# simplify23/TPS_PP

Hardware: AMD Instinct MI355X
Metric: rectified images/sec (3x32x100) (higher is better)
Workload: dtype f32; 1 GPU; BASELINE.json configs[1]: fused TPS grid-gen + bilinear grid_sample HIP kernel, batch 512 per GPU, 3x32x100 fp32, 20 fiducials, inputs resident in HBM; batch_per_gpu=512, rotating_buffer_sets=14, streams=3, repeats=1

## Files before the change

tps_pp_amd/csrc/tpspp_warp_pair.h:

```cpp
#pragma once
#include "tpspp_warp_dev.h"

namespace tpspp_pair {

using namespace tpspp_dev;

typedef float v4f __attribute__((ext_vector_type(4)));
typedef float v4f_a4 __attribute__((ext_vector_type(4), aligned(4)));
typedef __attribute__((address_space(1))) char gchar;

struct PairParams {
    const float* in; const float* ctrl; const float* inv_delta_c;
    const float* packed;
    const float* p_hat;
    int p_hat_ld;
    int N;
    float* out; float* grid; int32_t* idx;
    int zero_off;
    int out_off;
    long long* trace;
};

template <int F>
__device__ __forceinline__ constexpr int perm_y(int k) { return (k + F / 2) % F; }
template <int F>
__device__ __forceinline__ constexpr int perm_x(int k) { return k < F / 2 ? F / 2 - 1 - k : F + F / 2 - 1 - k; }

__device__ __forceinline__ void store16_nt(gchar* p, v4f v)
{
    asm volatile("global_store_dwordx4 %0, %1, off nt\n\ts_nop 1" ::"v"(p), "v"(v) : "memory");
}

__device__ __forceinline__ void wait_flag(const float* flag_word, int want)
{
    const volatile int* f = reinterpret_cast<const volatile int*>(flag_word);
    while (*f < want) __builtin_amdgcn_s_sleep(1);
}
__device__ __forceinline__ void wait_flag_lds(const float* flag_word, int want)
{
    typedef __attribute__((address_space(3))) const volatile int lds_cvint;
    lds_cvint* f = (lds_cvint*)(size_t)(unsigned)(size_t)flag_word;
    while (__builtin_amdgcn_readfirstlane(*f) < want) __builtin_amdgcn_s_sleep(1);
}

template <int OFF>
__device__ __forceinline__ void flag_add(unsigned addr, int one)
{
    asm volatile("ds_add_u32 %0, %1 offset:%2" ::"v"(addr), "v"(one), "n"(OFF) : "memory");
}

struct TapsLite {
    int o00;
    float nw, ne, sw, se;
    float wx, wy;
    bool inx, iny;
    int x0, y0;
};
__device__ __forceinline__ TapsLite make_taps_lite(float gx, float gy, int H, int W)
{
    TapsLite t;
    const float limx = (float)(W - 1), limy = (float)(H - 1);
    float ix = (gx + 1.0f) * (0.5f * limx);
    float iy = (gy + 1.0f) * (0.5f * limy);
    ix = (ix > 0.0f) ? ix : 0.0f;
    iy = (iy > 0.0f) ? iy : 0.0f;
    ix = __builtin_fminf(ix, limx);
    iy = __builtin_fminf(iy, limy);
    const float w = __builtin_amdgcn_fractf(ix), nn = __builtin_amdgcn_fractf(iy);
    int x0, y0;
    asm("v_cvt_flr_i32_f32 %0, %1" : "=v"(x0) : "v"(ix));
    asm("v_cvt_flr_i32_f32 %0, %1" : "=v"(y0) : "v"(iy));
    const float e = 1.0f - w, s = 1.0f - nn;
    t.nw = s * e; t.ne = s * w; t.sw = nn * e; t.se = nn * w;
    t.wx = w; t.wy = nn;
    t.inx = ix < limx;
    t.iny = iy < limy;
    t.o00 = __mul24(y0, W) + x0;
    t.x0 = x0; t.y0 = y0;
    return t;
}

template <int F, int q>
__device__ __forceinline__ void mirror_vals(const float* v_row, float (&val)[4])
{
    if constexpr (q == 0) {
        val[0] = val[1] = val[2] = val[3] = v_row[0];
    } else if constexpr (q == 1) {
        val[0] = v_row[1]; val[1] = -v_row[1]; val[2] = v_row[1]; val[3] = -v_row[1];
    } else if constexpr (q == 2) {
        val[0] = v_row[2]; val[1] = v_row[2]; val[2] = -v_row[2]; val[3] = -v_row[2];
    } else {
        constexpr int k = q - 3;
        val[0] = v_row[3 + k];
        val[1] = v_row[3 + perm_x<F>(k)];
        val[2] = v_row[3 + perm_y<F>(k)];
        val[3] = v_row[3 + perm_x<F>(perm_y<F>(k))];
    }
}

constexpr int kPairFlags = 4;
constexpr int kPairLoaders = 3;
constexpr int kPairAwait = 6;
constexpr int kPairKB = 4;

constexpr int kPairVarPacked = 1;
constexpr int kPairVarMfma = 2;
typedef float v2f __attribute__((ext_vector_type(2)));

template <int OH, int OW>
struct PairGeo {
    static constexpr int halfW = OW / 2;
    static constexpr int PW = (halfW + 3) & ~3;
    static constexpr int CGP = PW / 4;
    static constexpr int CG = (halfW - 2) / 4;
    static constexpr int SC0 = CG * 4;
    static constexpr int SW = OW - 2 * SC0;
    static constexpr int nthr = (OH / 2) * CG * 4;
    static constexpr int NW = nthr / kWave;
    static_assert(OW % 4 == 0 && (OH / 2) % 8 == 0 && nthr % kWave == 0, "needs whole 4 x 8 pixel blocks, whole wavefronts");
    static_assert(SW == 4 && OH * SW == 2 * kWave, "the centre strip is 4 columns, two wavefronts per image");
    static_assert(NW % 4 == 0 && NW >= 4, "the compute wavefronts spread evenly over the four SIMDs");
};
__host__ __device__ inline void pair_thread_pixel(int t, int CG, int* r, int* c)
{
    const int hw = t >> 5, l5 = t & 31, rg = hw / CG, cg = hw - rg * CG;
    *r = rg * 8 + (l5 >> 2);
    *c = cg * 4 + (l5 & 3);
}

template <int F, int C, int HC, int WC, int OH, int OW, bool AUX, bool TRACE, int VAR = 0>
__global__ void __launch_bounds__(1024)
tps_warp_pair_kernel(const PairParams P)
{
    using Geo = PairGeo<OH, OW>;
    constexpr int K = F + 3;
    constexpr int H = HC, W = WC;
    constexpr int NW = Geo::NW, NLOAD = kPairLoaders;
    constexpr int n = OH * OW;
    static_assert(NW + NLOAD <= 16, "too many wavefronts");
    extern __shared__ __attribute__((aligned(16))) float smem[];
    float4* sT = reinterpret_cast<float4*>(smem);
    float* sFlag = smem + 4 * K + 2 * ((K * K + 3) & ~3);
    float* sImg = sFlag + kPairFlags;
    float* sZero = sImg + P.zero_off;
    float* sOut = sImg + P.out_off;

    const int tid = threadIdx.x;
    const int lane = tid & (kWave - 1);
    const int wv = __builtin_amdgcn_readfirstlane(tid / kWave);
    const int b0 = blockIdx.x * 2;
    const bool hasB = (b0 + 1) < P.N;
    constexpr int HW = H * W;
    constexpr int img_elems = C * HW;

    unsigned ts[8];
#define PAIR_STAMP(i) do { if (TRACE) ts[i] = (unsigned)__builtin_amdgcn_s_memtime(); } while (0)
    long long wall0 = 0;
    if (TRACE) wall0 = (long long)wall_clock64();
    PAIR_STAMP(7);

    constexpr int KGI = (K + 3) / 4;
    float hrowv[KGI * 4];
    float cx = 0.0f, cy = 0.0f;
    if (wv < 2) {
        if (lane < F) {
            const int b = (wv == 1 && hasB) ? b0 + 1 : b0;
            const float2 cc = reinterpret_cast<const float2*>(P.ctrl + (size_t)b * F * 2)[lane];
            cx = cc.x; cy = cc.y;
        }
        const float* row = P.inv_delta_c + (lane < K ? lane : K - 1) * K;
#pragma unroll
        for (int j = 0; j < KGI; ++j) {
            const int c0 = (j == KGI - 1) ? K - 4 : 4 * j;
            const v4f_a4 x = *reinterpret_cast<const v4f_a4*>(row + c0);
            hrowv[4 * j] = x[0]; hrowv[4 * j + 1] = x[1]; hrowv[4 * j + 2] = x[2]; hrowv[4 * j + 3] = x[3];
        }
    }
    if (tid < kPairFlags) reinterpret_cast<int*>(sFlag)[tid] = 0;
    lds_only_barrier();

    if (wv >= NW) {
        const int lw = wv - NW;
        const int total_bytes = (hasB ? 2 : 1) * img_elems * 4;
        const int pieces = (total_bytes + 1023) >> 10;
        const int piecesA = (img_elems * 4 + 1023) >> 10;
        const char* src = reinterpret_cast<const char*>(P.in + (size_t)b0 * img_elems);
        auto dma = [&](int piece) {
            int off = piece * 1024 + lane * 16;
            if (off >= total_bytes) off = 0;
            __builtin_amdgcn_global_load_lds(
                (const __attribute__((address_space(1))) void*)(src + off),
                (__attribute__((address_space(3))) void*)(reinterpret_cast<char*>(sImg) + piece * 1024),
                16, 0, 2 );
        };
        unsigned fa = (unsigned)(size_t)(sFlag + 1), fb = (unsigned)(size_t)(sFlag + 2);
        int one = 1;
        asm volatile("" : "+v"(fa), "+v"(fb), "+v"(one));
        int piece = lw;
        for (; piece < piecesA; piece += NLOAD) dma(piece);
        asm volatile("s_waitcnt vmcnt(%0)" ::"n"(kPairAwait) : "memory");
#pragma unroll
        for (int i = 0; i < kPairKB; ++i) { if (piece < pieces) dma(piece); piece += NLOAD; }
        if (hasB) asm volatile("s_waitcnt vmcnt(%0)" ::"n"(kPairKB) : "memory");
        else      asm volatile("s_waitcnt vmcnt(0)" ::: "memory");
        if (lane == 0) flag_add<0>(fa, one);
        for (; piece < pieces; piece += NLOAD) dma(piece);
        asm volatile("s_waitcnt vmcnt(0)" ::: "memory");
        if (lane == 0) flag_add<0>(fb, one);
        return;
    }

    const int hw = tid >> 5, l5 = tid & 31;
    const int rg = hw / Geo::CG, cg = hw - rg * Geo::CG;
    const int r = rg * 8 + (l5 >> 2), c = cg * 4 + (l5 & 3);
    unsigned poff[4];
    poff[0] = 4u * (unsigned)(r * OW + c);
    poff[1] = 4u * (unsigned)(r * OW + (OW - 1 - c));
    poff[2] = 4u * (unsigned)((OH - 1 - r) * OW + c);
    poff[3] = 4u * (unsigned)((OH - 1 - r) * OW + (OW - 1 - c));
    const bool strip = wv < 4 && (wv < 2 || hasB);
    const int sim = wv >> 1;
    const int srow = (wv & 1) * (OH / 2) + (lane >> 2), scol = Geo::SC0 + (lane & 3);
    const unsigned spoff = 4u * (unsigned)(srow * OW + scol);

    constexpr int KG = (K + 3) / 4;
    float v[KG * 4];
    {
        const int t_old = (rg * Geo::CGP + cg) * 32 + l5;
        const v4f* pk = reinterpret_cast<const v4f*>(P.packed) + (size_t)(t_old >> 6) * KG * kWave + (t_old & (kWave - 1));
#pragma unroll
        for (int j = 0; j < KG; ++j) {
            const v4f x = pk[j * kWave];
            v[4 * j] = x[0]; v[4 * j + 1] = x[1]; v[4 * j + 2] = x[2]; v[4 * j + 3] = x[3];
        }
    }
    float u[KG * 4];
    if (wv < 4) {
        const float* row = P.p_hat + (size_t)(srow * OW + scol) * P.p_hat_ld;
#pragma unroll
        for (int j = 0; j < KG; ++j) {
            const v4f_a4 x = *reinterpret_cast<const v4f_a4*>(row + 4 * j);
            u[4 * j] = x[0]; u[4 * j + 1] = x[1]; u[4 * j + 2] = x[2]; u[4 * j + 3] = x[3];
        }
    }
    if (tid < C) sZero[tid * HW] = 0.0f;
    if (wv < 2) {
        float ax = 0.0f, ay = 0.0f;
        static_for<K>([&](auto qc) {
            constexpr int q = decltype(qc)::value;
            constexpr int idx = (q / 4 < KGI - 1) ? q : 4 * (KGI - 1) + (q - (K - 4));
            ax = fmaf(hrowv[idx], readlane_f(cx, q), ax);
            ay = fmaf(hrowv[idx], readlane_f(cy, q), ay);
        });
        if (lane < K) {
            float* dst = reinterpret_cast<float*>(sT + lane) + 2 * wv;
            dst[0] = ax; dst[1] = ay;
        }
        asm volatile("s_waitcnt lgkmcnt(0)" ::: "memory");
        if (lane == 0) __hip_atomic_fetch_add(reinterpret_cast<int*>(sFlag), 1, __ATOMIC_RELAXED, __HIP_MEMORY_SCOPE_WORKGROUP);
    }
    wait_flag_lds(sFlag + 0, 2);
    PAIR_STAMP(0);
    asm volatile("" ::"v"(v[KG * 4 - 1]), "v"(u[KG * 4 - 1]));

    float sgx = 0.0f, sgy = 0.0f;
    if (wv < 4) {
        static_for<K>([&](auto qc) {
            constexpr int q = decltype(qc)::value;
            const float2 t = reinterpret_cast<const float2*>(sT + q)[sim];
            sgx = fmaf(u[q], t.x, sgx);
            sgy = fmaf(u[q], t.y, sgy);
        });
        asm volatile("" : "+v"(sgx), "+v"(sgy));
    }

    float gx[4][2], gy[4][2];
#pragma unroll
    for (int m = 0; m < 4; ++m) gx[m][0] = gx[m][1] = gy[m][0] = gy[m][1] = 0.0f;
    if constexpr ((VAR & kPairVarMfma) != 0) {
        v4f macc[4];
#pragma unroll
        for (int m = 0; m < 4; ++m) macc[m] = v4f{0.0f, 0.0f, 0.0f, 0.0f};
        const float* tcomp = reinterpret_cast<const float*>(sT) + (lane & 3);
        static_for<K>([&](auto qc) {
            constexpr int q = decltype(qc)::value;
            const float tq = tcomp[4 * q];
            float val[4];
            if constexpr (q == 0) {
                val[0] = val[1] = val[2] = val[3] = v[0];
            } else if constexpr (q == 1) {
                val[0] = v[1]; val[1] = -v[1]; val[2] = v[1]; val[3] = -v[1];
            } else if constexpr (q == 2) {
                val[0] = v[2]; val[1] = v[2]; val[2] = -v[2]; val[3] = -v[2];
            } else {
                constexpr int k = q - 3;
                val[0] = v[3 + k];
                val[1] = v[3 + perm_x<F>(k)];
                val[2] = v[3 + perm_y<F>(k)];
                val[3] = v[3 + perm_x<F>(perm_y<F>(k))];
            }
#pragma unroll
            for (int m = 0; m < 4; ++m) macc[m] = __builtin_amdgcn_mfma_f32_4x4x1f32(tq, val[m], macc[m], 0, 0, 0);
        });
#pragma unroll
        for (int m = 0; m < 4; ++m) { gx[m][0] = macc[m][0]; gy[m][0] = macc[m][1]; gx[m][1] = macc[m][2]; gy[m][1] = macc[m][3]; }
    } else
    static_for<K>([&](auto qc) {
        constexpr int q = decltype(qc)::value;
        const float4 t = sT[q];
        float val[4];
        if constexpr (q == 0) {
            val[0] = val[1] = val[2] = val[3] = v[0];
        } else if constexpr (q == 1) {
            val[0] = v[1]; val[1] = -v[1]; val[2] = v[1]; val[3] = -v[1];
        } else if constexpr (q == 2) {
            val[0] = v[2]; val[1] = v[2]; val[2] = -v[2]; val[3] = -v[2];
        } else {
            constexpr int k = q - 3;
            val[0] = v[3 + k];
            val[1] = v[3 + perm_x<F>(k)];
            val[2] = v[3 + perm_y<F>(k)];
            val[3] = v[3 + perm_x<F>(perm_y<F>(k))];
        }
        if constexpr (VAR & kPairVarPacked) {
            const v2f tA = {t.x, t.y}, tB = {t.z, t.w};
#pragma unroll
            for (int m = 0; m < 4; ++m) {
                const v2f vv = {val[m], val[m]};
                v2f a = {gx[m][0], gy[m][0]}, b = {gx[m][1], gy[m][1]};
                a = __builtin_elementwise_fma(vv, tA, a);
                b = __builtin_elementwise_fma(vv, tB, b);
                gx[m][0] = a.x; gy[m][0] = a.y; gx[m][1] = b.x; gy[m][1] = b.y;
            }
        } else {
#pragma unroll
            for (int m = 0; m < 4; ++m) {
                gx[m][0] = fmaf(val[m], t.x, gx[m][0]);
                gy[m][0] = fmaf(val[m], t.y, gy[m][0]);
                gx[m][1] = fmaf(val[m], t.z, gx[m][1]);
                gy[m][1] = fmaf(val[m], t.w, gy[m][1]);
            }
        }
    });
#pragma unroll
    for (int m = 0; m < 4; ++m) asm volatile("" : "+v"(gx[m][0]), "+v"(gy[m][0]), "+v"(gx[m][1]), "+v"(gy[m][1]));

    constexpr unsigned row_bytes = n * 4u;
    constexpr int out16 = (C * n) >> 2;
    constexpr int nct = NW * kWave;
    typedef __attribute__((address_space(3))) const float lds_cfloat;
    const unsigned img_lds = (unsigned)(size_t)sImg, zero_lds = (unsigned)(size_t)sZero;
    auto describe_px = [&](float pgx, float pgy, int im, unsigned pix_off, bool st, unsigned (&a)[4], float (&w)[4]) {
        const TapsLite t = make_taps_lite(pgx, pgy, H, W);
        if constexpr (AUX) {
            const int b = b0 + im;
            if (P.grid && st)
                *reinterpret_cast<float2*>(reinterpret_cast<char*>(P.grid) + (size_t)b * 2 * row_bytes + 2u * pix_off) = make_float2(pgx, pgy);
            if (P.idx && st)
                *reinterpret_cast<int2*>(reinterpret_cast<char*>(P.idx) + (size_t)b * 2 * row_bytes + 2u * pix_off) = make_int2(t.x0, t.y0);
        }
        const unsigned a0 = img_lds + (unsigned)(im * img_elems * 4) + 4u * (unsigned)t.o00;
        a[0] = a0;
        a[1] = t.inx ? a0 + 4u : zero_lds;
        a[2] = t.iny ? a0 + 4u * W : zero_lds;
        a[3] = (t.inx && t.iny) ? a0 + 4u * W + 4u : zero_lds;
        w[0] = t.nw; w[1] = t.ne; w[2] = t.sw; w[3] = t.se;
    };
    unsigned ta[2][4][4];
    float tw[2][4][4];
#pragma unroll
    for (int im = 0; im < 2; ++im) {
#pragma unroll
        for (int m = 0; m < 4; ++m) describe_px(gx[m][im], gy[m][im], im, poff[m], im == 0 || hasB, ta[im][m], tw[im][m]);
#pragma unroll
        for (int m = 0; m < 4; ++m)
#pragma unroll
            for (int q = 0; q < 4; ++q) asm volatile("" : "+v"(ta[im][m][q]), "+v"(tw[im][m][q]));
    }
    unsigned sa[4] = {zero_lds, zero_lds, zero_lds, zero_lds};
    float sw[4] = {0.0f, 0.0f, 0.0f, 0.0f};
    if (wv < 4) describe_px(sgx, sgy, sim, spoff, strip, sa, sw);
    PAIR_STAMP(1);

    constexpr int NOUT = (out16 + nct - 1) / nct;
    v4f ostage[NOUT];
    auto store_image = [&](int b) {
        gchar* ob = (gchar*)(P.out) + (size_t)b * C * row_bytes;
#pragma unroll
        for (int i = 0; i < NOUT; ++i) {
            const int e = tid + i * nct;
            if (e < out16) store16_nt(ob + 16u * (unsigned)e, ostage[i]);
        }
    };
    auto read_staged = [&](const float* stage) {
#pragma unroll
        for (int i = 0; i < NOUT; ++i) {
            const int e = tid + i * nct;
            if (e < out16) ostage[i] = *reinterpret_cast<const v4f*>(reinterpret_cast<const char*>(stage) + 16 * e);
        }
    };
    auto load_taps = [&](int im, float (&tv)[4][C][4]) {
#pragma unroll
        for (int m = 0; m < 4; ++m)
#pragma unroll
            for (int ch = 0; ch < C; ++ch)
#pragma unroll
                for (int q = 0; q < 4; ++q) tv[m][ch][q] = *((lds_cfloat*)(size_t)(ta[im][m][q]) + ch * HW);
    };
    auto finish_image = [&](auto barc, int im, float (&tv)[4][C][4], bool mystrip, float* stage) {
        constexpr bool BAR = decltype(barc)::value;
        float res[4][C], sres[C];
#pragma unroll
        for (int m = 0; m < 4; ++m)
#pragma unroll
            for (int ch = 0; ch < C; ++ch) {
                float acc = tv[m][ch][0] * tw[im][m][0];
                acc = fmaf(tv[m][ch][1], tw[im][m][1], acc);
                acc = fmaf(tv[m][ch][2], tw[im][m][2], acc);
                acc = fmaf(tv[m][ch][3], tw[im][m][3], acc);
                res[m][ch] = acc;
            }
        if (mystrip) {
            __builtin_amdgcn_sched_barrier(0);
            float sv[C][4];
#pragma unroll
            for (int ch = 0; ch < C; ++ch)
#pragma unroll
                for (int q = 0; q < 4; ++q) sv[ch][q] = *((lds_cfloat*)(size_t)(sa[q]) + ch * HW);
#pragma unroll
            for (int ch = 0; ch < C; ++ch) {
                float acc = sv[ch][0] * sw[0];
                acc = fmaf(sv[ch][1], sw[1], acc);
                acc = fmaf(sv[ch][2], sw[2], acc);
                acc = fmaf(sv[ch][3], sw[3], acc);
                sres[ch] = acc;
            }
        }
        if (BAR) lds_only_barrier();
#pragma unroll
        for (int m = 0; m < 4; ++m)
#pragma unroll
            for (int ch = 0; ch < C; ++ch)
                *reinterpret_cast<float*>(reinterpret_cast<char*>(stage) + ch * (int)row_bytes + poff[m]) = res[m][ch];
        if (mystrip) {
#pragma unroll
            for (int ch = 0; ch < C; ++ch)
                *reinterpret_cast<float*>(reinterpret_cast<char*>(stage) + ch * (int)row_bytes + spoff) = sres[ch];
        }
    };

#pragma unroll
    for (int im = 0; im < 2; ++im) {
        if (im == 1 && !hasB) { store_image(b0); break; }
        wait_flag_lds(sFlag + 1 + im, NLOAD);
        PAIR_STAMP(2 + 2 * im);
        float tv[4][C][4];
        load_taps(im, tv);
        if (im == 1) {
            __builtin_amdgcn_sched_barrier(0);
            store_image(b0);
            __builtin_amdgcn_sched_barrier(0);
            finish_image(std::true_type{}, im, tv, strip && sim == im, sOut);
        } else {
            finish_image(std::false_type{}, im, tv, strip && sim == im, sOut);
        }
        lds_only_barrier();
        PAIR_STAMP(3 + 2 * im);
        read_staged(sOut);
        if (im == 1) {
            store_image(b0 + 1);
        } else {
            asm volatile("s_waitcnt lgkmcnt(0)" ::: "memory");
#pragma unroll
            for (int i = 0; i < NOUT; ++i) asm volatile("" : "+v"(ostage[i]));
        }
    }
    if (TRACE && wv == 0) {
        asm volatile("s_waitcnt vmcnt(0)" ::: "memory");
        PAIR_STAMP(6);
        if (lane == 0 && P.trace) {
            long long* t = P.trace + (size_t)blockIdx.x * 8;
            if (!hasB) ts[4] = ts[5] = ts[3];
#pragma unroll
            for (int i = 0; i < 7; ++i) t[i] = (long long)(ts[i] - ts[7]);
            t[7] = wall0;
        }
    }
#undef PAIR_STAMP
}


template <int F, int C, int HC, int WC, int OH, int OW>
inline size_t pair_lds_bytes(int* zero_off, int* out_off)
{
    constexpr int K = F + 3;
    const int pieces = (2 * C * HC * WC * 4 + 1023) / 1024;
    *zero_off = pieces * 256;
    *out_off = pieces * 256 + (C - 1) * HC * WC + 4;
    return (size_t)(4 * K + 2 * ((K * K + 3) & ~3) + kPairFlags) * sizeof(float) + (size_t)(*out_off) * 4 + (size_t)C * OH * OW * 4;
}

}
```

Before: 62.11 million images/s.

## Add per-channel software-pipelined tap loading variant and shrink LDS header

Adds an optional VAR-gated path that splits each image's bilinear tap gathers into channel units and double-buffers them, so the next unit's LDS loads are issued while the current unit is blended. It can also start the second image early if its loader flag is already set. It also drops the unused 2*K*K scratch region from the LDS layout, which shrinks shared memory per block and may raise occupancy. Adds trace-only arrival timestamps via LDS atomics. The default VAR is 0, so the pipelined path is inactive unless a caller selects it.

```diff
diff --git a/tps_pp_amd/csrc/tpspp_warp_pair.h b/tps_pp_amd/csrc/tpspp_warp_pair.h
--- a/tps_pp_amd/csrc/tpspp_warp_pair.h
+++ b/tps_pp_amd/csrc/tpspp_warp_pair.h
@@ -105,6 +105,9 @@
 
 constexpr int kPairVarPacked = 1;
 constexpr int kPairVarMfma = 2;
+constexpr int kPairVarPipe = 4;
+constexpr int kPairVarPipe2 = 8;
+constexpr int kPairVarLibrary = 0;
 typedef float v2f __attribute__((ext_vector_type(2)));
 
 template <int OH, int OW>
@@ -128,7 +131,7 @@
     *c = cg * 4 + (l5 & 3);
 }
 
-template <int F, int C, int HC, int WC, int OH, int OW, bool AUX, bool TRACE, int VAR = 0>
+template <int F, int C, int HC, int WC, int OH, int OW, bool AUX, bool TRACE, int VAR = kPairVarLibrary>
 __global__ void __launch_bounds__(1024)
 tps_warp_pair_kernel(const PairParams P)
 {
@@ -140,7 +143,7 @@
     static_assert(NW + NLOAD <= 16, "too many wavefronts");
     extern __shared__ __attribute__((aligned(16))) float smem[];
     float4* sT = reinterpret_cast<float4*>(smem);
-    float* sFlag = smem + 4 * K + 2 * ((K * K + 3) & ~3);
+    float* sFlag = smem + 4 * K;
     float* sImg = sFlag + kPairFlags;
     float* sZero = sImg + P.zero_off;
     float* sOut = sImg + P.out_off;
@@ -177,7 +180,11 @@
         }
     }
     if (tid < kPairFlags) reinterpret_cast<int*>(sFlag)[tid] = 0;
+    unsigned* sLate = reinterpret_cast<unsigned*>(sZero) + 1;
+    if (TRACE && tid == 0) { sLate[0] = ts[7]; sLate[1] = 0u; sLate[2] = 0u; }
     lds_only_barrier();
+#define PAIR_ARRIVE(i) do { if (TRACE) { const unsigned d_ = (unsigned)__builtin_amdgcn_s_memtime() - sLate[0]; \
+        if (lane == 0) __hip_atomic_fetch_max(sLate + (i), d_, __ATOMIC_RELAXED, __HIP_MEMORY_SCOPE_WORKGROUP); } } while (0)
 
     if (wv >= NW) {
         const int lw = wv - NW;
@@ -449,6 +456,112 @@
         }
     };
 
+    constexpr int UCH = (VAR & kPairVarPipe2) ? 2 : 1;
+    constexpr int UPI = (C + UCH - 1) / UCH;
+    auto issue_unit = [&](auto uc, float (&tq)[2][4][UCH][4], float (&ts4)[2][UCH][4]) {
+        constexpr int u = decltype(uc)::value, im = u / UPI, ch0 = (u % UPI) * UCH, nc = (C - ch0 < UCH) ? C - ch0 : UCH;
+#pragma unroll
+        for (int m = 0; m < 4; ++m)
+#pragma unroll
+            for (int q = 0; q < 4; ++q)
+#pragma unroll
+                for (int c = 0; c < nc; ++c) tq[u & 1][m][c][q] = *((lds_cfloat*)(size_t)(ta[im][m][q]) + (ch0 + c) * HW);
+        if (strip && sim == im) {
+#pragma unroll
+            for (int q = 0; q < 4; ++q)
+#pragma unroll
+                for (int c = 0; c < nc; ++c) ts4[u & 1][c][q] = *((lds_cfloat*)(size_t)(sa[q]) + (ch0 + c) * HW);
+        }
+    };
+    auto finish_unit = [&](auto uc, float (&tq)[2][4][UCH][4], float (&ts4)[2][UCH][4], float* stage) {
+        constexpr int u = decltype(uc)::value, im = u / UPI, ch0 = (u % UPI) * UCH, nc = (C - ch0 < UCH) ? C - ch0 : UCH;
+        const bool mystrip = strip && sim == im;
+        float res[4][UCH], sres[UCH];
+#pragma unroll
+        for (int m = 0; m < 4; ++m)
+#pragma unroll
+            for (int c = 0; c < nc; ++c) {
+                float acc = tq[u & 1][m][c][0] * tw[im][m][0];
+                acc = fmaf(tq[u & 1][m][c][1], tw[im][m][1], acc);
+                acc = fmaf(tq[u & 1][m][c][2], tw[im][m][2], acc);
+                acc = fmaf(tq[u & 1][m][c][3], tw[im][m][3], acc);
+                res[m][c] = acc;
+            }
+        if (mystrip) {
+#pragma unroll
+            for (int c = 0; c < nc; ++c) {
+                float acc = ts4[u & 1][c][0] * sw[0];
+                acc = fmaf(ts4[u & 1][c][1], sw[1], acc);
+                acc = fmaf(ts4[u & 1][c][2], sw[2], acc);
+                acc = fmaf(ts4[u & 1][c][3], sw[3], acc);
+                sres[c] = acc;
+            }
+        }
+        if constexpr (u == UPI) lds_only_barrier();
+#pragma unroll
+        for (int m = 0; m < 4; ++m)
+#pragma unroll
+            for (int c = 0; c < nc; ++c)
+                *reinterpret_cast<float*>(reinterpret_cast<char*>(stage) + (ch0 + c) * (int)row_bytes + poff[m]) = res[m][c];
+        if (mystrip) {
+#pragma unroll
+            for (int c = 0; c < nc; ++c)
+                *reinterpret_cast<float*>(reinterpret_cast<char*>(stage) + (ch0 + c) * (int)row_bytes + spoff) = sres[c];
+        }
+    };
+
+    if constexpr ((VAR & kPairVarPipe) != 0) {
+        float tq[2][4][UCH][4], ts4[2][UCH][4];
+        bool preB = false;
+        wait_flag_lds(sFlag + 1, NLOAD);
+        PAIR_STAMP(2);
+        issue_unit(std::integral_constant<int, 0>{}, tq, ts4);
+        static_for<UPI>([&](auto uc) {
+            constexpr int u = decltype(uc)::value;
+            if constexpr (u + 1 < UPI) {
+                issue_unit(std::integral_constant<int, u + 1>{}, tq, ts4);
+            } else {
+                typedef __attribute__((address_space(3))) const volatile int lds_cvint;
+                preB = hasB && __builtin_amdgcn_readfirstlane(*(lds_cvint*)(size_t)(unsigned)(size_t)(sFlag + 2)) >= NLOAD;
+                if (preB) {
+                    PAIR_STAMP(4);
+                    issue_unit(std::integral_constant<int, UPI>{}, tq, ts4);
+                }
+            }
+            __builtin_amdgcn_sched_barrier(0);
+            finish_unit(uc, tq, ts4, sOut);
+            __builtin_amdgcn_sched_barrier(0);
+        });
+        PAIR_ARRIVE(1);
+        lds_only_barrier();
+        PAIR_STAMP(3);
+        read_staged(sOut);
+        asm volatile("s_waitcnt lgkmcnt(0)" ::: "memory");
+#pragma unroll
+        for (int i = 0; i < NOUT; ++i) asm volatile("" : "+v"(ostage[i]));
+        if (hasB) {
+            if (!preB) {
+                wait_flag_lds(sFlag + 2, NLOAD);
+                PAIR_STAMP(4);
+                issue_unit(std::integral_constant<int, UPI>{}, tq, ts4);
+            }
+            static_for<UPI>([&](auto cc) {
+                constexpr int u = UPI + decltype(cc)::value;
+                if constexpr (u + 1 < 2 * UPI) issue_unit(std::integral_constant<int, u + 1>{}, tq, ts4);
+                __builtin_amdgcn_sched_barrier(0);
+                if constexpr (u == UPI) { store_image(b0); __builtin_amdgcn_sched_barrier(0); }
+                finish_unit(std::integral_constant<int, u>{}, tq, ts4, sOut);
+                __builtin_amdgcn_sched_barrier(0);
+            });
+            PAIR_ARRIVE(2);
+            lds_only_barrier();
+            PAIR_STAMP(5);
+            read_staged(sOut);
+            store_image(b0 + 1);
+        } else {
+            store_image(b0);
+        }
+    } else {
 #pragma unroll
     for (int im = 0; im < 2; ++im) {
         if (im == 1 && !hasB) { store_image(b0); break; }
@@ -464,6 +577,7 @@
         } else {
             finish_image(std::false_type{}, im, tv, strip && sim == im, sOut);
         }
+        PAIR_ARRIVE(1 + im);
         lds_only_barrier();
         PAIR_STAMP(3 + 2 * im);
         read_staged(sOut);
@@ -475,6 +589,7 @@
             for (int i = 0; i < NOUT; ++i) asm volatile("" : "+v"(ostage[i]));
         }
     }
+    }
     if (TRACE && wv == 0) {
         asm volatile("s_waitcnt vmcnt(0)" ::: "memory");
         PAIR_STAMP(6);
@@ -483,10 +598,13 @@
             if (!hasB) ts[4] = ts[5] = ts[3];
 #pragma unroll
             for (int i = 0; i < 7; ++i) t[i] = (long long)(ts[i] - ts[7]);
+            t[3] |= (long long)sLate[1] << 32;
+            t[5] |= (long long)(hasB ? sLate[2] : sLate[1]) << 32;
             t[7] = wall0;
         }
     }
 #undef PAIR_STAMP
+#undef PAIR_ARRIVE
 }
 
 
@@ -497,7 +615,7 @@
     const int pieces = (2 * C * HC * WC * 4 + 1023) / 1024;
     *zero_off = pieces * 256;
     *out_off = pieces * 256 + (C - 1) * HC * WC + 4;
-    return (size_t)(4 * K + 2 * ((K * K + 3) & ~3) + kPairFlags) * sizeof(float) + (size_t)(*out_off) * 4 + (size_t)C * OH * OW * 4;
-}
-
-}
+    return (size_t)(4 * K + kPairFlags) * sizeof(float) + (size_t)(*out_off) * 4 + (size_t)C * OH * OW * 4;
+}
+
+}
```

Result: no change. 62.19 million images/s (median of 2 runs) (+0.1%).
